# facebookresearch/dlrm

Hardware: NVIDIA H100
Metric: samples/sec (fwd+bwd) MLPerf-DLRM synthetic (higher is better)
Workload: dtype fp32 (bf16x3 split on wgmma, fp32 accumulate)

## Files before the change

### dlrm_b200/_lib.py

```python
import ctypes as C
import os

from . import _build

MAX_TABLES = 64
ACT_NONE, ACT_RELU, ACT_SIGMOID = 0, 1, 2
LOSS_MSE, LOSS_BCE, LOSS_WBCE = 0, 1, 2
OPT_SGD, OPT_RWSADAGRAD, OPT_ADAGRAD = 0, 1, 2
GEMM_SIMT_FP32, GEMM_TC_BF16X3, GEMM_TC_BF16 = 0, 1, 2
DTYPE_F32, DTYPE_F16 = 0, 1
TUNE = dict(emb_bags_per_group=0, emb_unroll=1, emb_block=2, upd_block=3, gemm_splitk=4, gemm_smem_kb=5,
            head_rows=6, interact_bwd_cols=7, pdl=8, chain_order=9, upd_lean=10, upd_debug=11)


class EmbFwdTable(C.Structure):
    _fields_ = [("weight", C.c_void_p), ("indices", C.c_void_p), ("offsets", C.c_void_p),
                ("row_weights", C.c_void_p), ("nnz", C.c_int64), ("rows", C.c_int64), ("ld", C.c_int64),
                ("out_off", C.c_int64), ("out_stride", C.c_int64), ("row_lo", C.c_int64), ("row_n", C.c_int64),
                ("weight_dtype", C.c_int32)]


class EmbBwdTable(C.Structure):
    _fields_ = [("weight", C.c_void_p), ("momentum", C.c_void_p), ("head", C.c_void_p),
                ("indices", C.c_void_p), ("offsets", C.c_void_p), ("nnz", C.c_int64),
                ("rows", C.c_int64), ("pair_base", C.c_int64), ("ld", C.c_int64), ("mom_stride", C.c_int64),
                ("use_dy_off", C.c_int64), ("dy_off", C.c_int64), ("row_lo", C.c_int64), ("row_n", C.c_int64),
                ("head_stride", C.c_int64), ("mark", C.c_void_p), ("weight_dtype", C.c_int32),
                ("round_key", C.c_uint64)]


class EmbRemoteTable(C.Structure):
    _fields_ = [("shard_weight", C.c_void_p * 8), ("num_shards", C.c_int32), ("rows_per_shard", C.c_int64),
                ("rows", C.c_int64), ("ld", C.c_int64), ("indices", C.c_void_p), ("offsets", C.c_void_p),
                ("nnz", C.c_int64), ("out_off", C.c_int64), ("out_stride", C.c_int64), ("weight_dtype", C.c_int32)]


class EmbDedup(C.Structure):
    _fields_ = [("filter", C.c_void_p), ("log2_size", C.c_int32), ("flags", C.c_void_p), ("suspects", C.c_void_p)]


class GemmTcDesc(C.Structure):
    _fields_ = [("A_hi", C.c_void_p), ("A_lo", C.c_void_p), ("lda", C.c_int64), ("a_mn_major", C.c_int),
                ("B_hi", C.c_void_p), ("B_lo", C.c_void_p), ("ldb", C.c_int64), ("b_mn_major", C.c_int),
                ("M", C.c_int64), ("N", C.c_int64), ("K", C.c_int64),
                ("mode_x3", C.c_int), ("split_k", C.c_int), ("tile_n", C.c_int), ("act", C.c_int),
                ("mask_act", C.c_int),
                ("mask_hi", C.c_void_p), ("mask_lo", C.c_void_p), ("ldmask", C.c_int64),
                ("out_f32", C.c_void_p), ("ld_f32", C.c_int64), ("slab_stride", C.c_int64),
                ("out_hi", C.c_void_p), ("out_lo", C.c_void_p), ("ld_out", C.c_int64),
                ("outT_hi", C.c_void_p), ("outT_lo", C.c_void_p), ("ld_outT", C.c_int64),
                ("out_col", C.c_void_p), ("col_index", C.c_int64), ("col_slab_stride", C.c_int64),
                ("bias", C.c_void_p)]


class DenseLayer(C.Structure):
    _fields_ = [("W", C.c_void_p), ("b", C.c_void_p), ("sW", C.c_void_p), ("sb", C.c_void_p),
                ("dW", C.c_void_p), ("db", C.c_void_p), ("pack_hi", C.c_void_p), ("pack_lo", C.c_void_p),
                ("slab_stride", C.c_int64), ("N", C.c_int64), ("K", C.c_int64), ("ld_pack", C.c_int64),
                ("num_slabs", C.c_int64)]


_lib = None

SYMBOLS = [
    "dlrm_b200_abi_version", "dlrm_b200_last_error", "dlrm_b200_device_info", "dlrm_b200_check_device_errors",
    "dlrm_b200_emb_bag_fwd", "dlrm_b200_emb_bag_fwd_train", "dlrm_b200_emb_bwd_link",
    "dlrm_b200_emb_bwd_update", "dlrm_b200_head_scratch_bytes", "dlrm_b200_head_fused",
    "dlrm_b200_interact_fwd_ex", "dlrm_b200_interact_bwd_ex", "dlrm_b200_interact_bwd_p2p", "dlrm_b200_act_bwd",
    "dlrm_b200_emb_bag_fwd_p2p", "dlrm_b200_emb_bwd_update_p2p", "dlrm_b200_emb_bwd_classify",
    "dlrm_b200_p2p_barrier", "dlrm_b200_p2p_allreduce_mean", "dlrm_b200_enable_peer_access",
    "dlrm_b200_ipc_export", "dlrm_b200_ipc_open", "dlrm_b200_ipc_close",
    "dlrm_b200_linear_fwd", "dlrm_b200_linear_dgrad", "dlrm_b200_linear_wgrad",
    "dlrm_b200_interact_fwd", "dlrm_b200_interact_bwd", "dlrm_b200_loss_fwd_bwd",
    "dlrm_b200_dense_update",
    "dlrm_b200_gemm_tc_plan_create", "dlrm_b200_gemm_tc_plan_info", "dlrm_b200_gemm_tc_run",
    "dlrm_b200_gemm_tc_plan_destroy", "dlrm_b200_gemm_chain_create", "dlrm_b200_gemm_chain_info",
    "dlrm_b200_gemm_chain_run", "dlrm_b200_gemm_chain_destroy", "dlrm_b200_gemm_chain_set_trace",
    "dlrm_b200_emb_bwd_small_scratch_bytes", "dlrm_b200_emb_bwd_small_update", "dlrm_b200_emb_reduce_partials",
    "dlrm_b200_block_copy", "dlrm_b200_gen_multihot", "dlrm_b200_set_tunable", "dlrm_b200_emb_bag_fwd_remote", "dlrm_b200_split_bf16", "dlrm_b200_dense_update_pack",
]


def _declare(lib):
    i64, i32, f32, vp = C.c_int64, C.c_int, C.c_float, C.c_void_p
    lib.dlrm_b200_abi_version.restype = i32
    lib.dlrm_b200_last_error.restype = C.c_char_p
    lib.dlrm_b200_set_tunable.argtypes = [i32, i32]
    lib.dlrm_b200_check_device_errors.argtypes = [vp]
    lib.dlrm_b200_device_info.argtypes = [i32, C.POINTER(i32), C.POINTER(i32), C.POINTER(i32)]
    lib.dlrm_b200_emb_bag_fwd.argtypes = [C.POINTER(EmbFwdTable), i32, i32, i64, i32, i32, vp, i64, i64, vp]
    lib.dlrm_b200_emb_bag_fwd_train.argtypes = [C.POINTER(EmbFwdTable), C.POINTER(EmbBwdTable), i32, i32, i64, i32,
                                                i32, vp, vp, i64, i64, C.POINTER(EmbDedup), vp]
    lib.dlrm_b200_emb_bwd_classify.argtypes = [C.POINTER(EmbBwdTable), i32, i64, i32, i32, vp, C.POINTER(EmbDedup), vp]
    lib.dlrm_b200_head_scratch_bytes.argtypes = [i64, i64]
# ... 159 lines not shown
```

### dlrm_b200/csrc/common.cuh

```cuda
#pragma once
#include <cuda_fp16.h>
#include <cuda_runtime.h>
#include <stdint.h>
#include <stdio.h>

#include "../../include/dlrm_b200.h"

namespace dlrm {

char* err_buf();
int set_error(const char* fmt, ...);
int get_tunable(int id);
unsigned* err_word_device();

enum Tunable {
  TUNE_EMB_BAGS_PER_GROUP = 0,
  TUNE_EMB_UNROLL = 1,
  TUNE_EMB_BLOCK = 2,
  TUNE_UPD_BLOCK = 3,
  TUNE_GEMM_SPLITK = 4,
  TUNE_GEMM_SMEM_KB = 5,
  TUNE_HEAD_ROWS = 6,
  TUNE_INTERACT_BWD_COLS = 7,
  TUNE_PDL = 8,
  TUNE_UPD_LEAN = 10,
  TUNE_UPD_DEBUG = 11,
  TUNE_CHAIN_ORDER = 9,
  TUNE_COUNT = 16
};

#define DLRM_CHECK_LAUNCH(name)                                                         \
  do {                                                                                  \
    cudaError_t e__ = cudaGetLastError();                                               \
    if (e__ != cudaSuccess)                                                             \
      return dlrm::set_error("%s: launch failed: %s", name, cudaGetErrorString(e__));   \
  } while (0)

#define DLRM_CUDA(call)                                                                 \
  do {                                                                                  \
    cudaError_t e__ = (call);                                                           \
    if (e__ != cudaSuccess)                                                             \
      return dlrm::set_error("%s failed: %s", #call, cudaGetErrorString(e__));          \
  } while (0)

__device__ __forceinline__ void pdl_launch_dependents() { asm volatile("griddepcontrol.launch_dependents;" ::: "memory"); }
__device__ __forceinline__ void pdl_wait() { asm volatile("griddepcontrol.wait;" ::: "memory"); }

template <typename... KArgs, typename... Args>
static inline cudaError_t launch_chain(void (*kernel)(KArgs...), dim3 grid, dim3 block, size_t smem,
                                       cudaStream_t st, Args&&... args) {
  cudaLaunchConfig_t cfg = {};
  cfg.gridDim = grid;
  cfg.blockDim = block;
  cfg.dynamicSmemBytes = smem;
  cfg.stream = st;
  cudaLaunchAttribute attr[1];
  attr[0].id = cudaLaunchAttributeProgrammaticStreamSerialization;
  attr[0].val.programmaticStreamSerializationAllowed = 1;
  cfg.attrs = attr;
  cfg.numAttrs = get_tunable(TUNE_PDL) == 2 ? 0 : 1;
  return cudaLaunchKernelEx(&cfg, kernel, static_cast<KArgs>(args)...);
}

static inline bool aligned16(const void* p) { return (reinterpret_cast<uintptr_t>(p) & 15) == 0; }

__device__ __forceinline__ float4 ldg_stream_f4(const float* p) {
  float4 v;
  asm("ld.global.nc.L1::no_allocate.v4.f32 {%0,%1,%2,%3}, [%4];"
               : "=f"(v.x), "=f"(v.y), "=f"(v.z), "=f"(v.w)
               : "l"(p));
  return v;
}

template <typename wt>
struct is_f16 { static constexpr bool value = false; };
template <>
struct is_f16<__half> { static constexpr bool value = true; };

__device__ __forceinline__ float4 h4_to_f4(uint2 u) {
  const float2 a = __half22float2(*reinterpret_cast<const __half2*>(&u.x));
  const float2 b = __half22float2(*reinterpret_cast<const __half2*>(&u.y));
  return make_float4(a.x, a.y, b.x, b.y);
}

template <typename wt>
__device__ __forceinline__ float4 ld_row4(const wt* p) {
  if constexpr (is_f16<wt>::value) return h4_to_f4(*reinterpret_cast<const uint2*>(p));
  else return *reinterpret_cast<const float4*>(p);
}
template <typename wt>
__device__ __forceinline__ float4 ldg_stream_row4(const wt* p) {
  if constexpr (is_f16<wt>::value) {
    uint2 u;
    asm("ld.global.nc.L1::no_allocate.v2.u32 {%0,%1}, [%2];" : "=r"(u.x), "=r"(u.y) : "l"(p));
    return h4_to_f4(u);
  } else {
    return ldg_stream_f4(p);
  }
}

__device__ __forceinline__ unsigned long long splitmix64(unsigned long long x) {
  x += 0x9E3779B97F4A7C15ull;
// ... 59 lines not shown
```

### dlrm_b200/csrc/emb_bwd.cu

```cuda
#include "common.cuh"

namespace dlrm {

__device__ __forceinline__ void list_walk_guard(unsigned& chunks, unsigned long long& t0) {
  if (++chunks >= 4096u && (chunks & 4095u) == 0u) {
    unsigned long long now;
    asm volatile("mov.u64 %0, %%globaltimer;" : "=l"(now));
    if (t0 == 0) t0 = now;
    else if (now - t0 > 20000000000ULL) {
      if ((threadIdx.x & 31) == 0) printf("dlrm_b200: emb update: a row's occurrence list does not end (stale list heads?)\n");
      __trap();
    }
  }
}

constexpr int LS_KEEP = 4;

struct ListWalk {
  const int2* link;
  int cur, self_bag;
  bool first;
  unsigned chunks;
  unsigned long long t0;
  __device__ __forceinline__ int chunk(int lane, int& bag) {
// ... 420 lines not shown
          sq = warp_sum(sq);
          const float m_new = m_old + sq * inv_d;
          const float stdv = sqrtf(m_new) + P.eps;
          const float nlr = -P.lr;
#pragma unroll
          for (int v = 0; v < NV; ++v)
            if (col_ok[v]) {
#pragma unroll
              for (int e = 0; e < W; ++e) w[v].x[e] = fmaf(nlr, g[v].x[e] / stdv, w[v].x[e]);
              st_pack<W>(wrow + lane * W + v * 32 * W, w[v], is_f16<wt>::value ? sr_bits(rkey, lane + 32 * v) : 0ull);
            }
          if (lane == 0) tb.mom[r * tb.mom_stride] = m_new;
        } else {
          const float nlr = -P.lr;
#pragma unroll
          for (int v = 0; v < NV; ++v)
            if (col_ok[v]) {
#pragma unroll
              for (int e = 0; e < W; ++e) w[v].x[e] = fmaf(nlr, g[v].x[e], w[v].x[e]);
              st_pack<W>(wrow + lane * W + v * 32 * W, w[v], is_f16<wt>::value ? sr_bits(rkey, lane + 32 * v) : 0ull);
            }
        }
        if (lane == 0 && ((susp_mask >> src) & 1u)) tb.head[r * tb.hs] = 0;
      }
    }
  }
}

struct UpdTableS {
  void* w;
  float* mom;
  int* head;
  unsigned char* mark;
  const void* idx;
  long long pair_base, ld, mom_stride, hs, dy_off, row_lo, row_n;
};

__device__ __noinline__ float4 upd_sum_long(const EmbBwdParams& P, int nxt, int self_bag, long long dy_off,
                                            bool col_ok) {
  const int lane = threadIdx.x & 31;
  auto load = [&](int bag, float (&t)[4]) {
    float4 v = make_float4(0.f, 0.f, 0.f, 0.f);
    if (col_ok) v = *reinterpret_cast<const float4*>(dy_row(P, bag) + dy_off + lane * 4);
    t[0] = v.x; t[1] = v.y; t[2] = v.z; t[3] = v.w;
  };
  float s[4];
  list_sum_exact<4>(P.link, nxt, self_bag, load, s);
  return make_float4(s[0], s[1], s[2], s[3]);
}

__device__ __noinline__ float4 upd_sum_duplicates(const EmbBwdParams& P, int nxt, int self_pos, int self_bag,
                                                  long long dy_off, int lane, bool col_ok) {
  float4 g = make_float4(0.f, 0.f, 0.f, 0.f);
  const int nxt0 = nxt;
  int cnt = 1;
  int mpos = (lane == 0) ? self_pos : 0x7fffffff;
  int mbag = self_bag;
  while (nxt != 0 && cnt < 32) {
    const int2 e = P.link[nxt - 1];
    if (lane == cnt) { mpos = nxt - 1; mbag = e.y; }
    ++cnt;
    nxt = e.x;
  }
  if (nxt != 0) return upd_sum_long(P, nxt0, self_bag, dy_off, col_ok);
  int rank = 0;
  for (int i = 0; i < cnt; ++i) rank += (__shfl_sync(0xffffffffu, mpos, i) < mpos) ? 1 : 0;
  constexpr int DUP_BATCH = 4;
  for (int q0 = 0; q0 < cnt; q0 += DUP_BATCH) {
    float4 t[DUP_BATCH];
#pragma unroll
    for (int u = 0; u < DUP_BATCH; ++u) {
      const unsigned who = __ballot_sync(0xffffffffu, lane < cnt && rank == q0 + u);
      const int bag = __shfl_sync(0xffffffffu, mbag, who ? __ffs(who) - 1 : 0);
      t[u] = (who && col_ok) ? *reinterpret_cast<const float4*>(dy_row(P, bag) + dy_off + lane * 4)
                             : make_float4(0.f, 0.f, 0.f, 0.f);
    }
#pragma unroll
    for (int u = 0; u < DUP_BATCH; ++u)
      if (q0 + u < cnt && col_ok) { g.x += t[u].x; g.y += t[u].y; g.z += t[u].z; g.w += t[u].w; }
  }
  return g;
}

template <typename wt, typename idx_t, int PF, int MINB, bool EW = false>
__global__ void __launch_bounds__(256, MINB) emb_update_lean_kernel(const __grid_constant__ EmbBwdParams P, int num_tables,
                                                                    long long total_hint) {
  __shared__ long long bound[DLRM_B200_MAX_TABLES_PER_CALL + 1], tend[DLRM_B200_MAX_TABLES_PER_CALL + 1];
  __shared__ UpdTableS ts[DLRM_B200_MAX_TABLES_PER_CALL];
  for (int k = threadIdx.x; k < num_tables; k += blockDim.x) {
    UpdTableS t;
    t.w = P.t[k].w; t.mom = P.t[k].mom; t.head = P.t[k].head; t.mark = P.t[k].mark; t.idx = P.t[k].idx;
    t.pair_base = P.t[k].pair_base; t.ld = P.t[k].ld; t.mom_stride = P.t[k].mom_stride; t.hs = P.t[k].hs;
    t.dy_off = P.t[k].dy_off; t.row_lo = P.t[k].row_lo; t.row_n = P.t[k].row_n;
    ts[k] = t;
  }
  load_bounds<idx_t>(bound, tend, P, num_tables, total_hint);
  const int D = P.dim;
  const int lane = threadIdx.x & 31;
  const int half = lane >> 4, l16 = lane & 15;
  const bool c0_ok = l16 * 8 < D, c1_ok = l16 * 8 + 4 < D;
  const bool col_ok = lane * 4 < D;
  const long long first = bound[0], total = bound[num_tables];
  const long long warp0 = (long long)blockIdx.x * (blockDim.x >> 5) + (threadIdx.x >> 5);
  const long long wstep = (long long)gridDim.x * (blockDim.x >> 5) * 32;
  const float inv_d = 1.0f / (float)D;
  const float nlr = -P.lr;
  const bool adagrad = !EW && P.optimizer == DLRM_OPT_RWSADAGRAD;
  const int dbg = P.debug;

  for (long long base = first + warp0 * 32; base < total; base += wstep) {
    const long long pos = base + lane;
    int k = table_of(bound, num_tables, base);
    if (base + 31 >= bound[k + 1]) k = table_of(bound, num_tables, pos < total ? pos : base);
    const UpdTableS& tb = ts[k];
    int r = 0;
    int2 lk = make_int2(0, 0);
    bool owner = false;
    if (pos < total && pos < tend[k] && tb.head != nullptr) {
      const long long rr = (long long)static_cast<const idx_t*>(tb.idx)[pos - tb.pair_base] - tb.row_lo;
      lk = P.link[pos];
      const unsigned char superseded = tb.mark[pos];
      if (superseded) tb.mark[pos] = 0;
      owner = (unsigned long long)rr < (unsigned long long)tb.row_n && !superseded;
      r = (int)rr;
    }
    const int nxt = owner ? lk.x : 0, bag = lk.y;
    wt* wptr = owner ? static_cast<wt*>(tb.w) + (long long)r * tb.ld : nullptr;
    const unsigned long long rkey =
        (is_f16<wt>::value && owner) ? sr_row_key(P.round_key[k], (long long)r + tb.row_lo) : 0ull;
    const float* gptr = owner ? dy_row(P, bag) + tb.dy_off : nullptr;
    float* mptr = (owner && (adagrad || EW)) ? tb.mom + (long long)r * tb.mom_stride : nullptr;
    int* hptr = owner ? tb.head + (long long)r * tb.hs : nullptr;
    unsigned simple = __ballot_sync(0xffffffffu, owner && nxt == 0);
    unsigned dups = __ballot_sync(0xffffffffu, owner && nxt != 0);

    while (simple) {
      float4 wv[PF][2], gv[PF][2];
      float4 sv[EW ? PF : 1][2];
      float mv[PF];
      int sa[PF], sb[PF];
#pragma unroll
      for (int u = 0; u < PF; ++u) {
        sa[u] = simple ? __ffs(simple) - 1 : -1;
        simple &= simple - 1u;
        sb[u] = simple ? __ffs(simple) - 1 : -1;
        simple &= simple - 1u;
        const int s_ = half ? sb[u] : sa[u];
        const int sc = s_ < 0 ? 0 : s_;
        const wt* wp = reinterpret_cast<const wt*>(__shfl_sync(0xffffffffu, (unsigned long long)wptr, sc)) + l16 * 8;
        const float* gp = reinterpret_cast<const float*>(__shfl_sync(0xffffffffu, (unsigned long long)gptr, sc)) + l16 * 8;
        const float4 z = make_float4(0.f, 0.f, 0.f, 0.f);
        const bool ldw = !(dbg & 2), ldg = !(dbg & 8);
        if constexpr (is_f16<wt>::value) {
          if (s_ >= 0 && c0_ok && ldw) {
            const uint4 h = *reinterpret_cast<const uint4*>(wp);
            wv[u][0] = h4_to_f4(make_uint2(h.x, h.y));
            wv[u][1] = h4_to_f4(make_uint2(h.z, h.w));
          } else {
            wv[u][0] = z; wv[u][1] = z;
          }
        } else {
          wv[u][0] = (s_ >= 0 && c0_ok && ldw) ? *reinterpret_cast<const float4*>(wp) : z;
          wv[u][1] = (s_ >= 0 && c1_ok && ldw) ? *reinterpret_cast<const float4*>(wp + 4) : z;
        }
        gv[u][0] = (s_ >= 0 && c0_ok && ldg) ? *reinterpret_cast<const float4*>(gp) : z;
        gv[u][1] = (s_ >= 0 && c1_ok && ldg) ? *reinterpret_cast<const float4*>(gp + 4) : z;
        mv[u] = (adagrad && (lane == sa[u] || lane == sb[u])) ? *mptr : 0.f;
        if constexpr (EW) {
          const float* sp = reinterpret_cast<const float*>(__shfl_sync(0xffffffffu, (unsigned long long)mptr, sc)) + l16 * 8;
// ... 91 lines not shown
          float sq = fmaf(g.x, g.x, fmaf(g.y, g.y, fmaf(g.z, g.z, g.w * g.w)));
          sq = warp_sum(sq);
          const float m_new = __shfl_sync(0xffffffffu, m_old, s_) + sq * inv_d;
          scale = nlr / (sqrtf(m_new) + P.eps);
          if (lane == s_) *mptr = m_new;
        }
        w.x = fmaf(scale, g.x, w.x); w.y = fmaf(scale, g.y, w.y);
        w.z = fmaf(scale, g.z, w.z); w.w = fmaf(scale, g.w, w.w);
      }
      if constexpr (is_f16<wt>::value) {
        const unsigned long long rk = __shfl_sync(0xffffffffu, rkey, s_);
        if (col_ok) st_row4(wp + lane * 4, w, sr_bits(rk, lane));
      } else {
        if (col_ok) *reinterpret_cast<float4*>(wp + lane * 4) = w;
      }
      if (lane == s_) *hptr = 0;
    }
  }
}

static int fill_params(EmbBwdParams& P, const dlrm_emb_bwd_table_t* tables, int num_tables,
                       const char* who) {
  if (num_tables < 0 || num_tables > DLRM_B200_MAX_TABLES_PER_CALL)
    return set_error("%s: num_tables=%d out of range [0,%d]", who, num_tables,
                     DLRM_B200_MAX_TABLES_PER_CALL);
  for (int k = 0; k < num_tables; ++k) {
    if (!tables[k].offsets || (!tables[k].indices && tables[k].nnz > 0))
      return set_error("%s: table %d has a NULL pointer", who, k);
    if (tables[k].pair_base + tables[k].nnz > 0x7ffffffeLL)
      return set_error("%s: more than 2^31-2 index occurrences in one call", who);
    P.t[k].w = tables[k].weight;
    P.t[k].mom = tables[k].momentum;
    P.t[k].head = tables[k].head;
    P.t[k].mark = tables[k].mark;
    if (tables[k].head && !tables[k].mark) return set_error("%s: table %d: head without a mark array", who, k);
    P.t[k].idx = tables[k].indices;
    P.t[k].off = tables[k].offsets;
    P.t[k].nnz = tables[k].nnz;
    P.t[k].pair_base = tables[k].pair_base;
    P.t[k].ld = tables[k].ld;
    P.t[k].mom_stride = tables[k].mom_stride > 0 ? tables[k].mom_stride : 1;
    P.t[k].hs = tables[k].head_stride > 0 ? tables[k].head_stride : 1;
    P.t[k].dy_off = 0;
    P.t[k].rows = tables[k].rows > 0 ? tables[k].rows : 0x7fffffffffffffffLL;
    P.t[k].row_lo = tables[k].row_n > 0 ? tables[k].row_lo : 0;
    P.t[k].row_n = tables[k].row_n > 0 ? tables[k].row_n : P.t[k].rows;
    P.round_key[k] = tables[k].round_key;
    if (tables[k].weight_dtype != tables[0].weight_dtype)
      return set_error("%s: table %d: weight_dtype differs from table 0's (one row type per call)", who, k);
  }
  if (num_tables > 0 && tables[0].weight_dtype != DLRM_DTYPE_F32 && tables[0].weight_dtype != DLRM_DTYPE_F16)
    return set_error("%s: weight_dtype=%d", who, tables[0].weight_dtype);
  return 0;
}

}

extern "C" int dlrm_b200_emb_bwd_link(const dlrm_emb_bwd_table_t* tables, int num_tables,
                                      int64_t batch, int idx_bytes, int include_last,
                                      int32_t* next, void* stream) {
  using namespace dlrm;
  EmbBwdParams P{};
  if (int rc = fill_params(P, tables, num_tables, "emb_bwd_link")) return rc;
  if (idx_bytes != 4 && idx_bytes != 8) return set_error("emb_bwd_link: idx_bytes=%d", idx_bytes);
  if (num_tables == 0 || batch == 0) return 0;
  if (!next) return set_error("emb_bwd_link: next is NULL");
  P.link = reinterpret_cast<int2*>(next);
  P.batch = batch;
  P.include_last = include_last;
  long long max_nnz = 0;
  for (int k = 0; k < num_tables; ++k) max_nnz = tables[k].nnz > max_nnz ? tables[k].nnz : max_nnz;
  if (max_nnz == 0) return 0;
  const int block = 256;
  long long gx = (max_nnz + block - 1) / block;
  if (gx > 65535) gx = 65535;
  dim3 grid((unsigned)gx, (unsigned)num_tables);
  cudaStream_t st = static_cast<cudaStream_t>(stream);
  if (idx_bytes == 8) emb_link_kernel<long long><<<grid, block, 0, st>>>(P);
  else emb_link_kernel<int><<<grid, block, 0, st>>>(P);
  DLRM_CHECK_LAUNCH("emb_link_kernel");
  return 0;
}

constexpr int EW_PF = 2, EW_MINB = 2;

static int emb_update_impl(const dlrm_emb_bwd_table_t* tables, int num_tables, int dim, int64_t batch,
                           int idx_bytes, int include_last, const int32_t* next, const float* dY,
                           int64_t dy_stride_sample, int64_t dy_stride_table, int optimizer, float lr,
                           float eps, void* stream, const float* const* peer_dY, int world,
                           int64_t batch_local, const dlrm_emb_dedup_t* dedup) {
  using namespace dlrm;
  EmbBwdParams P{};
  if (int rc = fill_params(P, tables, num_tables, "emb_bwd_update")) return rc;
  if (idx_bytes != 4 && idx_bytes != 8) return set_error("emb_bwd_update: idx_bytes=%d", idx_bytes);
  if (optimizer != DLRM_OPT_SGD && optimizer != DLRM_OPT_RWSADAGRAD && optimizer != DLRM_OPT_ADAGRAD)
    return set_error("emb_bwd_update: optimizer=%d", optimizer);
  const bool ew = optimizer == DLRM_OPT_ADAGRAD;
  if (dim <= 0 || dim > 1024) return set_error("emb_bwd_update: dim=%d unsupported (1..1024)", dim);
  const bool f16 = num_tables > 0 && tables[0].weight_dtype == DLRM_DTYPE_F16;
  if (f16 && dim % 8) return set_error("emb_bwd_update: fp16 tables need dim %% 8 == 0 (dim=%d)", dim);
  bool lean_rows = true;
  if (num_tables == 0 || batch == 0) return 0;
  if (!next || (!dY && !peer_dY)) return set_error("emb_bwd_update: NULL next/dY");
  bool vec = (dim % 4 == 0) && (peer_dY || aligned16(dY)) && dy_stride_sample % 4 == 0 && dy_stride_table % 4 == 0;
  P.flags = (dedup && dedup->flags) ? dedup->flags : nullptr;
  P.peer_batch = 0;
  for (int d = 0; d < DLRM_B200_MAX_PEERS; ++d) P.peer_dY[d] = nullptr;
  if (peer_dY) {
    if (world < 1 || world > DLRM_B200_MAX_PEERS || batch_local <= 0 || batch_local * world != batch)
      return set_error("emb_bwd_update_p2p: world=%d batch_local=%lld batch=%lld", world, (long long)batch_local,
                       (long long)batch);
    for (int d = 0; d < world; ++d) {
      if (!peer_dY[d]) return set_error("emb_bwd_update_p2p: peer %d pointer is NULL", d);
      vec = vec && aligned16(peer_dY[d]);
      P.peer_dY[d] = peer_dY[d];
    }
    P.peer_batch = batch_local;
    dY = peer_dY[0];
  }
  for (int k = 0; k < num_tables; ++k) {
    P.t[k].dy_off = tables[k].use_dy_off ? tables[k].dy_off : (int64_t)k * dy_stride_table;
    vec = vec && (P.t[k].dy_off % 4 == 0);
    if (!tables[k].weight) return set_error("emb_bwd_update: table %d weight NULL", k);
    if ((optimizer == DLRM_OPT_RWSADAGRAD || ew) && !tables[k].momentum)
      return set_error("emb_bwd_update: table %d momentum NULL", k);
    if (ew) {
      P.t[k].mom_stride = tables[k].mom_stride > 0 ? tables[k].mom_stride : dim;
      if (P.t[k].mom_stride < dim) return set_error("emb_bwd_update: table %d: Adagrad mom_stride < dim", k);
      vec = vec && aligned16(tables[k].momentum) && P.t[k].mom_stride % 4 == 0;
    }
    vec = vec && aligned16(tables[k].weight);
    if (P.t[k].ld <= 0) P.t[k].ld = dim;
    if (P.t[k].ld < dim) return set_error("emb_bwd_update: table %d: ld < dim", k);
    vec = vec && (P.t[k].ld % 4 == 0);
    lean_rows = lean_rows && (!f16 || P.t[k].ld % 8 == 0);
  }
  P.link = reinterpret_cast<int2*>(const_cast<int32_t*>(next));
  P.dY = dY;
  P.dy_stride_sample = dy_stride_sample;
  P.dy_stride_table = dy_stride_table;
  P.batch = batch;
  P.dim = dim;
  P.include_last = include_last;
  P.optimizer = optimizer;
  P.lr = lr;
  P.eps = eps;
  P.debug = get_tunable(TUNE_UPD_DEBUG);
  const int block = 256;
  long long total = 0;
  for (int k = 0; k < num_tables; ++k) total += tables[k].nnz;
  if (include_last) {
    total = 0;
    for (int k = 0; k < num_tables; ++k) total = tables[k].nnz > total ? tables[k].nnz : total;
  }
  if (total == 0) return 0;
  int dev = 0, sms = 0;
  DLRM_CUDA(cudaGetDevice(&dev));
  DLRM_CUDA(cudaDeviceGetAttribute(&sms, cudaDevAttrMultiProcessorCount, dev));
  long long gridx = (total / 32 + block / 32) / (block / 32);
  if (gridx > (long long)sms * 3) gridx = (long long)sms * 3;
  if (gridx < 1) gridx = 1;
  const long long total_hint = include_last ? 0 : (tables[num_tables - 1].pair_base + tables[num_tables - 1].nnz);
  cudaStream_t st = static_cast<cudaStream_t>(stream);
#define UPD_E(WT, Wd, NV, EW)                                                                                \
  do {                                                                                                           \
    if (idx_bytes == 8)                                                                                          \
      emb_update_kernel<WT, Wd, NV, long long, EW><<<(unsigned)gridx, block, 0, st>>>(P, num_tables, total_hint); \
    else                                                                                                         \
      emb_update_kernel<WT, Wd, NV, int, EW><<<(unsigned)gridx, block, 0, st>>>(P, num_tables, total_hint);      \
    DLRM_CHECK_LAUNCH("emb_update_kernel");                                                                      \
    return 0;                                                                                                    \
  } while (0)
#define UPD_T(WT, Wd, NV)   \
  do {                      \
    if (ew) UPD_E(WT, Wd, NV, true); \
    UPD_E(WT, Wd, NV, false);        \
  } while (0)
#define UPD(Wd, NV) UPD_T(float, Wd, NV)
#define LEAN(WT, IDX)                                                                                              \
  do {                                                                                                             \
    if (ew) emb_update_lean_kernel<WT, IDX, EW_PF, EW_MINB, true><<<(unsigned)gl, block, 0, st>>>(P, num_tables, total_hint); \
    else emb_update_lean_kernel<WT, IDX, 2, 3><<<(unsigned)gl, block, 0, st>>>(P, num_tables, total_hint);        \
  } while (0)
  if (f16 && !vec)
    return set_error("emb_bwd_update: fp16 tables need a 16-byte aligned weight pointer, ld %% 4 == 0 (8-byte rows) "
                     "and 16-byte aligned gradient rows%s", ew ? " and accumulators (momentum, mom_stride % 4 == 0)" : "");
  if (vec && lean_rows && dim <= 128 && !P.flags && get_tunable(TUNE_UPD_LEAN) != 2) {
    long long gl = (total / 32 + block / 32) / (block / 32);
    if (gl > (long long)sms * 3) gl = (long long)sms * 3;
    if (gl < 1) gl = 1;
    if (f16) {
      if (idx_bytes == 8) LEAN(__half, long long);
      else LEAN(__half, int);
    } else if (idx_bytes == 8) {
      LEAN(float, long long);
    } else {
      LEAN(float, int);
    }
    DLRM_CHECK_LAUNCH("emb_update_lean_kernel");
    return 0;
  }
  if (f16) {
    if (dim <= 128) UPD_T(__half, 4, 1);
    if (dim <= 256) UPD_T(__half, 4, 2);
    if (dim <= 512) UPD_T(__half, 4, 4);
    UPD_T(__half, 4, 8);
  }
  if (vec) {
    if (dim <= 128) UPD(4, 1);
    if (dim <= 256) UPD(4, 2);
    if (dim <= 512) UPD(4, 4);
    UPD(4, 8);
  }
  if (dim <= 32) UPD(1, 1);
  if (dim <= 64) UPD(1, 2);
  if (dim <= 128) UPD(1, 4);
  if (dim <= 256) UPD(1, 8);
  if (dim <= 512) UPD(1, 16);
  UPD(1, 32);
#undef LEAN
#undef UPD
#undef UPD_T
#undef UPD_E
}

extern "C" int dlrm_b200_emb_bwd_update(const dlrm_emb_bwd_table_t* tables, int num_tables, int dim,
                                        int64_t batch, int idx_bytes, int include_last,
                                        const int32_t* next, const float* dY,
                                        int64_t dy_stride_sample, int64_t dy_stride_table,
                                        int optimizer, float lr, float eps, const dlrm_emb_dedup_t* dedup,
                                        void* stream) {
  return emb_update_impl(tables, num_tables, dim, batch, idx_bytes, include_last, next, dY, dy_stride_sample,
                         dy_stride_table, optimizer, lr, eps, stream, nullptr, 0, 0, dedup);
}

extern "C" int dlrm_b200_emb_bwd_classify(const dlrm_emb_bwd_table_t* tables, int num_tables, int64_t batch,
                                          int idx_bytes, int include_last, int32_t* next,
                                          const dlrm_emb_dedup_t* dedup, void* stream) {
  using namespace dlrm;
  EmbBwdParams P{};
  if (int rc = fill_params(P, tables, num_tables, "emb_bwd_classify")) return rc;
  if (idx_bytes != 4 && idx_bytes != 8) return set_error("emb_bwd_classify: idx_bytes=%d", idx_bytes);
  if (!dedup || !dedup->filter || !dedup->flags || !dedup->suspects || !next)
    return set_error("emb_bwd_classify: NULL dedup buffers");
  if (num_tables == 0 || batch == 0) return 0;
  P.link = reinterpret_cast<int2*>(next);
  P.batch = batch;
  P.include_last = include_last;
  long long total = 0;
  for (int k = 0; k < num_tables; ++k) total += tables[k].nnz;
  if (include_last) {
    total = 0;
    for (int k = 0; k < num_tables; ++k) total = tables[k].nnz > total ? tables[k].nnz : total;
  }
  if (total == 0) return 0;
  const long long total_hint = include_last ? 0 : (tables[num_tables - 1].pair_base + tables[num_tables - 1].nnz);
  int dev = 0, sms = 0;
  DLRM_CUDA(cudaGetDevice(&dev));
  DLRM_CUDA(cudaDeviceGetAttribute(&sms, cudaDevAttrMultiProcessorCount, dev));
  long long gridx = (total / 32 + 7) / 8;
  if (gridx > (long long)sms * 8) gridx = (long long)sms * 8;
  if (gridx < 1) gridx = 1;
  cudaStream_t st = static_cast<cudaStream_t>(stream);
  int* n_susp = reinterpret_cast<int*>(dedup->filter + ((size_t)1 << dedup->log2_size));
  if (idx_bytes == 8) {
    emb_classify_kernel<long long><<<(unsigned)gridx, 256, 0, st>>>(P, num_tables, total_hint, dedup->filter,
                                                                    dedup->log2_size, dedup->flags, dedup->suspects, n_susp);
    DLRM_CHECK_LAUNCH("emb_classify_kernel");
    emb_link_suspects_kernel<long long><<<sms, 256, 0, st>>>(P, num_tables, total_hint, dedup->suspects, n_susp);
  } else {
    emb_classify_kernel<int><<<(unsigned)gridx, 256, 0, st>>>(P, num_tables, total_hint, dedup->filter,
                                                              dedup->log2_size, dedup->flags, dedup->suspects, n_susp);
// ... 19 lines not shown
```

### dlrm_b200/engine.py

```python
from __future__ import annotations

import contextlib
import ctypes as C
import os
from dataclasses import dataclass
from typing import List, Optional, Sequence

import numpy as np
import torch

from . import _lib
from ._lib import (ACT_NONE, ACT_RELU, ACT_SIGMOID, DTYPE_F16, DTYPE_F32, GEMM_SIMT_FP32, LOSS_BCE, LOSS_MSE,
                   LOSS_WBCE, OPT_ADAGRAD, OPT_RWSADAGRAD, OPT_SGD, EmbBwdTable, EmbFwdTable)

_LOSS = {"mse": LOSS_MSE, "bce": LOSS_BCE, "wbce": LOSS_WBCE}
_OPT = {"sgd": OPT_SGD, "rwsadagrad": OPT_RWSADAGRAD, "adagrad": OPT_ADAGRAD}
_LR_DECAY = ("rwsadagrad", "adagrad")


def _ptr(t: Optional[torch.Tensor]) -> Optional[int]:
    return None if t is None else t.data_ptr()


def _stream() -> int:
# ... 880 lines not shown
                self.tc_splits[(which, i)] = sk
                smax = max(smax, sk)
        if self.dense_grad.numel() < smax * P:
            self.dense_grad = torch.zeros(smax * P, dtype=torch.float32, device=dev)
            self.dW, self.db = {"bot": [], "top": []}, {"bot": [], "top": []}
            for name, i, kind, o, shape in self.dense_slices:
                n = int(np.prod(shape))
                (self.dW if kind == "W" else self.db)[name].append(self.dense_grad[o:o + n].view(shape))
        self._dense_off = {}
        for name, i, kind, o, shape in self.dense_slices:
            self._dense_off[(name, i, kind)] = o
        for which in ("bot", "top"):
            ln = self.ln_bot if which == "bot" else self.ln_top
            ntc = self.ntc[which]
            ins, gzs, Ws = [], [], []
            for i in range(ntc):
                K, N = ln[i], ln[i + 1]
                Kp, Np = r8(K + 1), r8(N)
                h = torch.zeros((B, Kp), dtype=bf, device=dev)
                l = torch.zeros((B, Kp), dtype=bf, device=dev)
                h[:, K] = 1.0
                ins.append((h, l, Kp))
                gzs.append((torch.zeros((B, Np), dtype=bf, device=dev), torch.zeros((B, Np), dtype=bf, device=dev), Np))
                Ws.append((torch.zeros((N, Kp), dtype=bf, device=dev), torch.zeros((N, Kp), dtype=bf, device=dev), Kp))
            self.tc_in[which], self.tc_gz[which], self.tc_W[which] = ins, gzs, Ws
        FD = self.F * self.D
        fwd_kb = int(os.environ.get("DLRM_TC_FWD_SMEM_KB", self.tc_smem_kb[0]))
        bwd_kb = int(os.environ.get("DLRM_TC_BWD_SMEM_KB", self.tc_smem_kb[1]))

        def GP(_kb, **kw):
            if "tile_n" not in kw:
                kw["tile_n"] = int(os.environ.get("DLRM_CHAIN_TILE_N", "0"))
            _lib.set_tunable("gemm_smem_kb", _kb)
            try:
                return _lib.GemmTcPlan(**kw)
            finally:
                _lib.set_tunable("gemm_smem_kb", 0)

        for which in ("bot", "top"):
            ln = self.ln_bot if which == "bot" else self.ln_top
            ntc = self.ntc[which]
            nl = len(ln) - 1
            for i in range(ntc):
                K, N = ln[i], ln[i + 1]
                ih, il, Kp = self.tc_in[which][i]
                wh, wl, _ = self.tc_W[which][i]
                gh, gl, Np = self.tc_gz[which][i]
                kw = dict(A_hi=ih.data_ptr(), A_lo=il.data_ptr(), lda=Kp, a_mn_major=0,
                          B_hi=wh.data_ptr(), B_lo=wl.data_ptr(), ldb=Kp, b_mn_major=0,
                          M=B, N=N, K=K, mode_x3=x3, split_k=1, act=self._act(which, i),
                          bias=self.b[which][i].data_ptr())
                if i + 1 < ntc:
                    oh, ol, Kp2 = self.tc_in[which][i + 1]
                    kw.update(out_hi=oh.data_ptr(), out_lo=ol.data_ptr(), ld_out=Kp2)
                if which == "bot" and i == nl - 1:
                    kw.update(out_f32=self.Tbuf.data_ptr(), ld_f32=FD)
                elif which == "top" and (i == ntc - 1):
                    kw.update(out_f32=self.top_act[i].data_ptr(), ld_f32=self.top_act[i].shape[1])
                self.tc_plans["fwd"][(which, i)] = GP(fwd_kb, **kw)
                oW = self._dense_off[(which, i, "W")]
                ob = self._dense_off[(which, i, "b")]
                self.tc_plans["wgrad"][(which, i)] = GP(
                    bwd_kb, A_hi=gh.data_ptr(), A_lo=gl.data_ptr(), lda=Np, a_mn_major=1,
                    B_hi=ih.data_ptr(), B_lo=il.data_ptr(), ldb=Kp, b_mn_major=1,
                    M=N, N=K + 1, K=B, mode_x3=x3, split_k=self.tc_splits[(which, i)],
                    out_f32=self.dense_grad.data_ptr() + oW * 4, ld_f32=K, slab_stride=P,
                    out_col=self.dense_grad.data_ptr() + ob * 4, col_index=K, col_slab_stride=P)
                if i > 0:
                    ph, pl, Np_prev = self.tc_gz[which][i - 1]
                    self.tc_plans["dgrad"][(which, i)] = GP(
                        bwd_kb, A_hi=gh.data_ptr(), A_lo=gl.data_ptr(), lda=Np, a_mn_major=0,
                        B_hi=wh.data_ptr(), B_lo=wl.data_ptr(), ldb=Kp, b_mn_major=1,
                        M=B, N=K, K=N, mode_x3=x3, split_k=1,
                        mask_act=self._act(which, i - 1), mask_hi=ih.data_ptr(), mask_lo=il.data_ptr(), ldmask=Kp,
                        out_hi=ph.data_ptr(), out_lo=pl.data_ptr(), ld_out=Np_prev)
                elif which == "top" and self.op == "dot":
                    self.tc_plans["dgrad"][(which, 0)] = GP(
                        bwd_kb, A_hi=gh.data_ptr(), A_lo=gl.data_ptr(), lda=Np, a_mn_major=0,
                        B_hi=wh.data_ptr(), B_lo=wl.data_ptr(), ldb=Kp, b_mn_major=1,
                        M=B, N=K, K=N, mode_x3=x3, split_k=1,
                        out_f32=self.dR.data_ptr(), ld_f32=self.ldr)
        if self.use_chain:
            self._build_chains()
        self._pack_dirty = True

    def _split(self, x: torch.Tensor, ldx: int, M: int, N: int, hl):
        h, l, ld = hl
        _lib.check(self.lib.dlrm_b200_split_bf16(x.data_ptr(), ldx, M, N, h.data_ptr(), l.data_ptr(), ld,
                                                 _stream()), "split_bf16")
        self.n_launch += 1

    def _dense_update_pack(self, opt_code: int, lr: float, eps: float = 1e-10, single_slab: bool = False):
        layers = []
        P = self.dense_numel
        for which in ("bot", "top"):
            ln = self.ln_bot if which == "bot" else self.ln_top
            for i in range(len(ln) - 1):
                d = _lib.DenseLayer()
                oW, ob = self._dense_off[(which, i, "W")], self._dense_off[(which, i, "b")]
                d.W = self.dense.data_ptr() + oW * 4
                d.b = self.dense.data_ptr() + ob * 4
                if self.dense_state is not None:
                    d.sW = self.dense_state.data_ptr() + oW * 4
                    d.sb = self.dense_state.data_ptr() + ob * 4
                d.dW = self.dense_grad.data_ptr() + oW * 4
                d.db = self.dense_grad.data_ptr() + ob * 4
                d.slab_stride = P
                d.N, d.K = ln[i + 1], ln[i]
                if i < self.ntc[which]:
                    wh, wl, Kp = self.tc_W[which][i]
                    d.pack_hi, d.pack_lo, d.ld_pack = wh.data_ptr(), wl.data_ptr(), Kp
                    d.num_slabs = self.tc_splits[(which, i)] if (opt_code >= 0 or opt_code == -2) and not single_slab else 1
                else:
                    d.num_slabs = 1
                layers.append(d)
        for c0 in range(0, len(layers), 16):
            chunk = layers[c0:c0 + 16]
            arr = (_lib.DenseLayer * len(chunk))(*chunk)
            _lib.check(self.lib.dlrm_b200_dense_update_pack(arr, len(chunk), opt_code, lr, eps, _stream()),
                       "dense_update_pack")
            self.n_launch += 1

    def _tc_prepare(self, B: int):
        if self.tc_B != B:
            self._tc_setup(B)
        if self._pack_dirty:
            self._dense_update_pack(-1, 0.0)
            self._pack_dirty = False

    def _tc_mlp_forward(self, which: str, B: int, skip_head: bool = False):
        ln = self.ln_bot if which == "bot" else self.ln_top
        s = _stream()
        ntc = self.ntc[which]
        if self.use_chain and ntc:
            self.tc_chains[("fwd", which)].run(s)
            self.n_launch += 1
        else:
            for i in range(ntc):
                self.tc_plans["fwd"][(which, i)].run(s)
                self.n_launch += 1
        nl = len(ln) - 1
        if which == "top" and self.has_head:
            nl -= 1
            if not skip_head:
                self._head(B, None, False)
        for i in range(ntc, nl):
            K, N = ln[i], ln[i + 1]
            x = self.top_act[i - 1]
            _lib.check(self.lib.dlrm_b200_linear_fwd(x.data_ptr(), x.shape[1], self.W[which][i].data_ptr(), K,
                                                     self.b[which][i].data_ptr(), self.top_act[i].data_ptr(),
                                                     self.top_act[i].shape[1], B, N, K, self._act(which, i),
                                                     GEMM_SIMT_FP32, s), "linear_fwd")
            self.n_launch += 1

    def _tc_forward(self, X: torch.Tensor, sp: SparseInput, link: bool = False, skip_head: bool = False) -> torch.Tensor:
        B = X.shape[0]
        self._tc_prepare(B)
        if self.ntc["bot"] == 0 or self.ntc["top"] == 0 or self.op != "dot":
            raise RuntimeError("gemm='tc' needs op='dot' and MLP layers of width >= 16; use gemm='simt'")
        FD = self.F * self.D
        ms = self.multi_stream and (self.T > 0 or self.gather_fn is not None)
        self._mark("begin")
        if ms:
            self._fork(self.s_emb)
            with torch.cuda.stream(self.s_emb):
                if self.gather_fn is not None:
                    self.gather_fn(sp, link)
                else:
                    self.emb_forward(sp, link=link)
                    self._mark("emb:gather")
                    self.reduce_partials(B)
                    self._mark("emb:reduce_partials")
        self._split(X, X.stride(0), B, self.ln_bot[0], self.tc_in["bot"][0])
        self._tc_mlp_forward("bot", B)
        self._mark("bot_fwd")
        if ms:
            self._join(self.s_emb)
            self._mark("join_gather")
        elif self.gather_fn is not None:
            self.gather_fn(sp, link)
        elif self.T:
            ev = self._gather_events
            if ev is not None:
                ev[0].record()
            self.emb_forward(sp, link=link)
            self.reduce_partials(B)
            if ev is not None:
                ev[1].record()
        rh, rl, ldrb = self.tc_in["top"][0]
        if self.D % 4 == 0:
            _lib.check(self.lib.dlrm_b200_interact_fwd_ex(self.Tbuf.data_ptr(), FD, None, self.ldr, rh.data_ptr(),
                                                          rl.data_ptr(), ldrb, B, self.F, self.D, int(self.itself),
                                                          _stream()), "interact_fwd_ex")
            self.n_launch += 1
        else:
            _lib.check(self.lib.dlrm_b200_interact_fwd(self.Tbuf.data_ptr(), FD, self.Rbuf.data_ptr(), self.ldr, B,
                                                       self.F, self.D, int(self.itself), _stream()), "interact_fwd")
            self.n_launch += 1
            self._split(self.Rbuf, self.ldr, B, self.num_int, self.tc_in["top"][0])
        self._mark("interact_fwd")
        self._tc_mlp_forward("top", B, skip_head)
        self._mark("top_fwd")
        p = self.top_act[-1][:B]
        if 0.0 < self.loss_threshold < 1.0:
            return torch.clamp(p, self.loss_threshold, 1.0 - self.loss_threshold)
        return p

    def _tc_mlp_backward(self, which: str, B: int):
        if self.use_chain:
            self.tc_chains[("bwd", which)].run(_stream())
            self.n_launch += 1
            return
        for i in reversed(range(self.ntc[which])):
            if self.multi_stream:
                self._fork(self.s_wg)
                with torch.cuda.stream(self.s_wg):
                    self.tc_plans["wgrad"][(which, i)].run(_stream())
            else:
                self.tc_plans["wgrad"][(which, i)].run(_stream())
            self.n_launch += 1
            pl = self.tc_plans["dgrad"].get((which, i))
            if pl is not None:
                pl.run(_stream())
                self.n_launch += 1

    def _build_chains(self):
        self.tc_chains, self._chain_ctr = {}, {}
        for which in ("bot", "top"):
            ntc = self.ntc[which]
            if ntc == 0:
                continue
            plans = [self.tc_plans["fwd"][(which, i)] for i in range(ntc)]
            self._make_chain(("fwd", which), plans, [-1] + list(range(ntc - 1)), [0] * ntc)
            plans, dep, onk = [], [], []
            producer = {}
            prev = -1
            for i in reversed(range(ntc)):
                producer[i] = prev
                pl = self.tc_plans["dgrad"].get((which, i))
                if pl is not None:
                    plans.append(pl); dep.append(prev); onk.append(0)
                    prev = len(plans) - 1
                else:
                    prev = -1
            for i in reversed(range(ntc)):
                plans.append(self.tc_plans["wgrad"][(which, i)]); dep.append(producer[i]); onk.append(1)
            self._make_chain(("bwd", which), plans, dep, onk)

    def _make_chain(self, key, plans, dep, onk):
        ctr = torch.zeros(_lib.GemmChain.counters_needed(plans), dtype=torch.int32, device=self.device)
        self._chain_ctr[key] = ctr
        self.tc_chains[key] = _lib.GemmChain(plans, dep, onk, ctr)

    def _tc_backward(self, X: torch.Tensor, sp: SparseInput, target: torch.Tensor, update=None):
        B = X.shape[0]
        FD = self.F * self.D
        s = _stream()
        nt, ntc = len(self.ln_top) - 1, self.ntc["top"]
        top_ld = [t.shape[1] for t in self.top_act]
        head_to_tc = False
        if getattr(self, "_external_gz", False):
            pass
        elif self.has_head:
            self._head(B, target, True)
            head_to_tc = (nt - 2) < ntc
            nt -= 1
        else:
            self.loss_and_grad(target, B)
        for i in reversed(range(ntc, nt)):
            K, N = self.ln_top[i], self.ln_top[i + 1]
            xin = self.top_act[i - 1]
            _lib.check(self.lib.dlrm_b200_linear_wgrad(self.top_gz[i].data_ptr(), top_ld[i], xin.data_ptr(),
                                                       xin.shape[1], self.dW["top"][i].data_ptr(), K,
                                                       self.db["top"][i].data_ptr(), B, N, K, GEMM_SIMT_FP32, s),
                       "linear_wgrad")
            _lib.check(self.lib.dlrm_b200_linear_dgrad(self.top_gz[i].data_ptr(), top_ld[i],
                                                       self.W["top"][i].data_ptr(), K, xin.data_ptr(),
                                                       xin.shape[1], self._act("top", i - 1),
                                                       self.top_gz[i - 1].data_ptr(), top_ld[i - 1], B, N, K,
                                                       GEMM_SIMT_FP32, s), "linear_dgrad")
            self.n_launch += 3
        if not head_to_tc:
            self._split(self.top_gz[ntc - 1], top_ld[ntc - 1], B, self.ln_top[ntc], self.tc_gz["top"][ntc - 1])
        self._mark("head+loss")
        self._tc_mlp_backward("top", B)
        self._mark("top_bwd_dgrad")
        bot_last_act = self._act("bot", len(self.ln_bot) - 2)
        g0h, g0l, ldg0 = self.tc_gz["bot"][-1]
        if self.dT_route is not None:
            self._interact_bwd_routed(B, bot_last_act, g0h.data_ptr(), g0l.data_ptr(), ldg0, s)
        else:
            _lib.check(self.lib.dlrm_b200_interact_bwd_ex(self.Tbuf.data_ptr(), FD, self.dR.data_ptr(), self.ldr,
                                                          self.dT.data_ptr(), FD, B, self.F, self.D,
                                                          int(self.itself), bot_last_act, g0h.data_ptr(),
                                                          g0l.data_ptr(), ldg0, s),
                       "interact_bwd_ex")
        self.n_launch += 1
        self._mark("interact_bwd")
        has_emb = self.T > 0 or self.update_fn is not None
        if update is not None and has_emb:
            opt, clr = update
            upd = (lambda: self.update_fn(sp, opt, clr)) if self.update_fn is not None else \
                (lambda: self.emb_update(sp, optimizer=opt, lr=clr))
            if self.multi_stream:
                self._fork(self.s_emb)
                with torch.cuda.stream(self.s_emb):
                    upd()
                    self._mark("emb:update")
            else:
                upd()
                self._mark("emb:update")
        self._tc_mlp_backward("bot", B)
        self._mark("bot_bwd_dgrad")
        if self.multi_stream:
            if not self.use_chain:
                self._join(self.s_wg)
                self._mark("join_wgrads")
            if update is not None and has_emb and getattr(self, "_join_update", True):
                self._join(self.s_emb)
                self._mark("join_update")


def _refuse_graphed_f16(eng: "Engine"):
    if eng.f16:
        raise RuntimeError("fp16 embedding tables train with eager steps: a captured training step would replay one "
                           "step's stochastic-rounding bits on every replay")


class GraphedTrainSteps:

    def __init__(self, eng: "Engine", stages, lr: float, optimizer: str = "rwsadagrad", warmup: int = 2):
        _refuse_graphed_f16(eng)
        self.eng, self.stages, self.lr, self.optimizer = eng, list(stages), lr, optimizer
        self.K = len(self.stages)
        eng.ensure_optimizer_state(optimizer)
        self.losses = torch.zeros(self.K, dtype=torch.float32, device=eng.device)
        side = torch.cuda.Stream()
        side.wait_stream(torch.cuda.current_stream())
        with torch.cuda.stream(side):
            for _ in range(max(warmup, 1)):
                self._eager()
        torch.cuda.current_stream().wait_stream(side)
        torch.cuda.synchronize()
        n0 = eng.n_launch
        self.graph = torch.cuda.CUDAGraph()
        with torch.cuda.graph(self.graph):
            self._eager()
        self.kernels_per_replay = eng.n_launch - n0

    def _eager(self):
        for j, st in enumerate(self.stages):
            loss = self.eng.train_step(st.X, st.sparse, st.target, self.lr, self.optimizer,
                                       join_update=(j == self.K - 1))
            self.losses[j:j + 1].copy_(loss)
        return self.losses

    def replay(self):
        self.graph.replay()
        self.eng.n_launch += self.kernels_per_replay
        self.eng.opt_step += self.K
        return self.losses


class GraphedTrainStep:

    def __init__(self, eng: "Engine", stage, lr: float, optimizer: str = "rwsadagrad", warmup: int = 3,
                 train: bool = True, X: Optional[torch.Tensor] = None, target: Optional[torch.Tensor] = None,
                 pre=None):
        if train:
            _refuse_graphed_f16(eng)
        self.eng, self.stage, self.train, self.pre = eng, stage, train, pre
        self.X = X if X is not None else stage.X
        self.target = target if target is not None else stage.target
        self.lr, self.optimizer = lr, optimizer
        eng.ensure_optimizer_state(optimizer)
        if warmup > 0:
            side = torch.cuda.Stream()
            side.wait_stream(torch.cuda.current_stream())
            with torch.cuda.stream(side):
                for _ in range(warmup):
                    self._eager()
            torch.cuda.current_stream().wait_stream(side)
        else:
            eng.prepare(stage.sparse, train, batch=self.X.shape[0])
        torch.cuda.synchronize()
        n0 = eng.n_launch
        self.graph = torch.cuda.CUDAGraph()
        with torch.cuda.graph(self.graph):
            self.out = self._eager()
        self.kernels_per_replay = eng.n_launch - n0

    def _eager(self):
        st = self.stage
        if self.pre is not None:
# ... 25 lines not shown
```

Baseline: 2.778 million.

## Defer top-MLP wgrads past interaction backward and resize lean update kernel grid

When every top-MLP dgrad plan already launches enough CTAs to fill the GPU, the top-layer weight-gradient GEMMs are deferred until after the interaction backward and embedding update are issued. This keeps the critical dgrad path from competing with wgrads for SMs. Separately, the lean embedding-update kernel now uses large fixed-size blocks (768 or 512 threads, one block per SM) instead of a min-blocks launch bound with up to 3 blocks per SM, and a tunable can override the grid size. The risks are lower occupancy from the larger blocks and less overlap for wgrads that are deferred.

```diff
diff --git a/dlrm_b200/_lib.py b/dlrm_b200/_lib.py
--- a/dlrm_b200/_lib.py
+++ b/dlrm_b200/_lib.py
@@ -9,7 +9,7 @@
 OPT_SGD, OPT_RWSADAGRAD, OPT_ADAGRAD = 0, 1, 2
 GEMM_SIMT_FP32, GEMM_TC_BF16X3, GEMM_TC_BF16 = 0, 1, 2
 DTYPE_F32, DTYPE_F16 = 0, 1
-TUNE = dict(emb_bags_per_group=0, emb_unroll=1, emb_block=2, upd_block=3, gemm_splitk=4, gemm_smem_kb=5,
+TUNE = dict(emb_bags_per_group=0, emb_unroll=1, emb_block=2, upd_grid=3, gemm_splitk=4, gemm_smem_kb=5,
             head_rows=6, interact_bwd_cols=7, pdl=8, chain_order=9, upd_lean=10, upd_debug=11)
 
 
diff --git a/dlrm_b200/csrc/common.cuh b/dlrm_b200/csrc/common.cuh
--- a/dlrm_b200/csrc/common.cuh
+++ b/dlrm_b200/csrc/common.cuh
@@ -17,7 +17,7 @@
   TUNE_EMB_BAGS_PER_GROUP = 0,
   TUNE_EMB_UNROLL = 1,
   TUNE_EMB_BLOCK = 2,
-  TUNE_UPD_BLOCK = 3,
+  TUNE_UPD_GRID = 3,
   TUNE_GEMM_SPLITK = 4,
   TUNE_GEMM_SMEM_KB = 5,
   TUNE_HEAD_ROWS = 6,
diff --git a/dlrm_b200/csrc/emb_bwd.cu b/dlrm_b200/csrc/emb_bwd.cu
--- a/dlrm_b200/csrc/emb_bwd.cu
+++ b/dlrm_b200/csrc/emb_bwd.cu
@@ -526,9 +526,9 @@
   return g;
 }
 
-template <typename wt, typename idx_t, int PF, int MINB, bool EW = false>
-__global__ void __launch_bounds__(256, MINB) emb_update_lean_kernel(const __grid_constant__ EmbBwdParams P, int num_tables,
-                                                                    long long total_hint) {
+template <typename wt, typename idx_t, int PF, int NT, bool EW = false>
+__global__ void __launch_bounds__(NT, 1) emb_update_lean_kernel(const __grid_constant__ EmbBwdParams P, int num_tables,
+                                                                long long total_hint) {
   __shared__ long long bound[DLRM_B200_MAX_TABLES_PER_CALL + 1], tend[DLRM_B200_MAX_TABLES_PER_CALL + 1];
   __shared__ UpdTableS ts[DLRM_B200_MAX_TABLES_PER_CALL];
   for (int k = threadIdx.x; k < num_tables; k += blockDim.x) {
@@ -786,7 +786,7 @@
   return 0;
 }
 
-constexpr int EW_PF = 2, EW_MINB = 2;
+constexpr int LEAN_PF = 2, LEAN_NT = 768, EW_PF = 2, EW_NT = 512;
 
 static int emb_update_impl(const dlrm_emb_bwd_table_t* tables, int num_tables, int dim, int64_t batch,
                            int idx_bytes, int include_last, const int32_t* next, const float* dY,
@@ -883,15 +883,17 @@
 #define UPD(Wd, NV) UPD_T(float, Wd, NV)
 #define LEAN(WT, IDX)                                                                                              \
   do {                                                                                                             \
-    if (ew) emb_update_lean_kernel<WT, IDX, EW_PF, EW_MINB, true><<<(unsigned)gl, block, 0, st>>>(P, num_tables, total_hint); \
-    else emb_update_lean_kernel<WT, IDX, 2, 3><<<(unsigned)gl, block, 0, st>>>(P, num_tables, total_hint);        \
+    if (ew) emb_update_lean_kernel<WT, IDX, EW_PF, EW_NT, true><<<(unsigned)gl, EW_NT, 0, st>>>(P, num_tables, total_hint); \
+    else emb_update_lean_kernel<WT, IDX, LEAN_PF, LEAN_NT><<<(unsigned)gl, LEAN_NT, 0, st>>>(P, num_tables, total_hint); \
   } while (0)
   if (f16 && !vec)
     return set_error("emb_bwd_update: fp16 tables need a 16-byte aligned weight pointer, ld %% 4 == 0 (8-byte rows) "
                      "and 16-byte aligned gradient rows%s", ew ? " and accumulators (momentum, mom_stride % 4 == 0)" : "");
   if (vec && lean_rows && dim <= 128 && !P.flags && get_tunable(TUNE_UPD_LEAN) != 2) {
-    long long gl = (total / 32 + block / 32) / (block / 32);
-    if (gl > (long long)sms * 3) gl = (long long)sms * 3;
+    const int warps = (ew ? EW_NT : LEAN_NT) / 32;
+    long long gl = (total / 32 + warps) / warps;
+    if (gl > sms) gl = sms;
+    if (get_tunable(TUNE_UPD_GRID) > 0) gl = get_tunable(TUNE_UPD_GRID);
     if (gl < 1) gl = 1;
     if (f16) {
       if (idx_bytes == 8) LEAN(__half, long long);
diff --git a/dlrm_b200/engine.py b/dlrm_b200/engine.py
--- a/dlrm_b200/engine.py
+++ b/dlrm_b200/engine.py
@@ -986,6 +986,7 @@
                         out_f32=self.dR.data_ptr(), ld_f32=self.ldr)
         if self.use_chain:
             self._build_chains()
+        self._tc_defer_top_wgrads = self._tc_dgrads_fill_gpu("top")
         self._pack_dirty = True
 
     def _split(self, x: torch.Tensor, ldx: int, M: int, N: int, hl):
@@ -1110,23 +1111,38 @@
             return torch.clamp(p, self.loss_threshold, 1.0 - self.loss_threshold)
         return p
 
-    def _tc_mlp_backward(self, which: str, B: int):
+    def _tc_mlp_backward(self, which: str, B: int, wgrads: bool = True):
         if self.use_chain:
             self.tc_chains[("bwd", which)].run(_stream())
             self.n_launch += 1
             return
         for i in reversed(range(self.ntc[which])):
-            if self.multi_stream:
-                self._fork(self.s_wg)
-                with torch.cuda.stream(self.s_wg):
-                    self.tc_plans["wgrad"][(which, i)].run(_stream())
-            else:
-                self.tc_plans["wgrad"][(which, i)].run(_stream())
-            self.n_launch += 1
+            if wgrads:
+                self._tc_wgrad(which, i)
             pl = self.tc_plans["dgrad"].get((which, i))
             if pl is not None:
                 pl.run(_stream())
                 self.n_launch += 1
+
+    def _tc_mlp_wgrads(self, which: str):
+        if self.use_chain:
+            return
+        for i in reversed(range(self.ntc[which])):
+            self._tc_wgrad(which, i)
+
+    def _tc_dgrads_fill_gpu(self, which: str) -> bool:
+        sms = torch.cuda.get_device_properties(self.device).multi_processor_count
+        ctas = [pl.info()["ctas"] for (w, _), pl in self.tc_plans["dgrad"].items() if w == which]
+        return bool(ctas) and min(ctas) >= sms
+
+    def _tc_wgrad(self, which: str, i: int):
+        if self.multi_stream:
+            self._fork(self.s_wg)
+            with torch.cuda.stream(self.s_wg):
+                self.tc_plans["wgrad"][(which, i)].run(_stream())
+        else:
+            self.tc_plans["wgrad"][(which, i)].run(_stream())
+        self.n_launch += 1
 
     def _build_chains(self):
         self.tc_chains, self._chain_ctr = {}, {}
@@ -1187,7 +1203,8 @@
         if not head_to_tc:
             self._split(self.top_gz[ntc - 1], top_ld[ntc - 1], B, self.ln_top[ntc], self.tc_gz["top"][ntc - 1])
         self._mark("head+loss")
-        self._tc_mlp_backward("top", B)
+        defer = self._tc_defer_top_wgrads
+        self._tc_mlp_backward("top", B, wgrads=not defer)
         self._mark("top_bwd_dgrad")
         bot_last_act = self._act("bot", len(self.ln_bot) - 2)
         g0h, g0l, ldg0 = self.tc_gz["bot"][-1]
@@ -1214,6 +1231,8 @@
             else:
                 upd()
                 self._mark("emb:update")
+        if defer:
+            self._tc_mlp_wgrads("top")
         self._tc_mlp_backward("bot", B)
         self._mark("bot_bwd_dgrad")
         if self.multi_stream:
```

Result: faster. 2.906 million, median of 6 (+4.6%).
